# mathisbot/homomorph-rust

Hardware: AMD Instinct MI355X
Metric: homomorphic u32 ops/sec (add, mul) at d=dp=tau=128; 1/2/4/8 MI355X (higher is better)
Workload: dtype u32

## Files before the change

homomorph-rust_amd/csrc/adder_mfma.hip:

```cpp
#include <hip/hip_runtime.h>

#include "mfma_gf2.h"

namespace hm {

#ifdef HM_MFMA_PROFILE
constexpr int kMfmaProfSlots = 8;
__device__ unsigned long long *g_mfma_prof;
#define HM_PT(v) const unsigned long long v = __builtin_amdgcn_s_memtime()
#define HM_PACC(k, a, b) prof[k] += (b) - (a)
#else
#define HM_PT(v)
#define HM_PACC(k, a, b)
#endif

#ifndef HM_MFMA_PREFETCH
#define HM_MFMA_PREFETCH 3
#endif
#ifndef HM_MFMA_PREFETCH25
#define HM_MFMA_PREFETCH25 4
#endif
template <int NC> constexpr int kPrefetchOf = NC > 16 ? HM_MFMA_PREFETCH25 : NC <= 8 ? 2 : HM_MFMA_PREFETCH;
template <int NC> constexpr int kStage(int k) { return NC <= 8 ? 2 * k : 1 + 3 * k; }
template <int NC, class Side, int kPrefetch = kPrefetchOf<NC>>
__device__ __forceinline__ v16f tile_mfma(const v8i (&Af)[NC], uint32_t rb, uint32_t rbn,
                                          u32x4 (&pf)[kPrefetch], v16f acc, Side &&side) {
    static_assert(NC - kPrefetch > kStage<NC>(2), "next tile's B reads must follow its ring fill (stage 2)");
    u32x4 bq[NC];
#pragma unroll
    for (int c = 0; c < kPrefetch; ++c) bq[c] = pf[c];
#pragma unroll
    for (int c = 0; c < NC; ++c) {
        if (c + kPrefetch < NC) bq[c + kPrefetch] = lds_at<const u32x4>(rb)[2 * (c + kPrefetch)];
        else pf[c + kPrefetch - NC] = lds_at<const u32x4>(rbn)[2 * (c + kPrefetch - NC)];
        const v8i Bf = {(int)bq[c].x, (int)bq[c].y, (int)bq[c].z, (int)bq[c].w, 0, 0, 0, 0};
        acc = mfma_fp4(Af[c], Bf, acc);
        asm volatile("" : "+v"(acc)::"memory");
        if (c == kStage<NC>(0)) side(0);
        if (c == kStage<NC>(1)) side(1);
        if (c == kStage<NC>(2)) side(2);
    }
    return acc;
}

constexpr uint32_t kPhaseBytes = 16u * 32u;

#ifndef HM_REC_WAIT_YOUNG
#define HM_REC_WAIT_YOUNG 0
#endif
__device__ __forceinline__ void wait_record(int young) {
    if (!HM_REC_WAIT_YOUNG || young <= 0) asm volatile("s_waitcnt vmcnt(0)" ::: "memory");
    else if (young >= 16) asm volatile("s_waitcnt vmcnt(16)" ::: "memory");
    else if (young >= 8) asm volatile("s_waitcnt vmcnt(8)" ::: "memory");
    else if (young >= 4) asm volatile("s_waitcnt vmcnt(4)" ::: "memory");
    else if (young >= 2) asm volatile("s_waitcnt vmcnt(2)" ::: "memory");
    else asm volatile("s_waitcnt vmcnt(1)" ::: "memory");
}

__device__ __forceinline__ void sum_store(uint64_t base, uint32_t off, uint32_t v) {
    asm volatile("global_store_dword %0, %1, %2" : : "v"(off), "v"(v), "s"(base) : "memory");
}

constexpr int kGetregHwId = 4 | 31 << 11;
constexpr int kGetregWaveSlot = 4 | 3 << 11;
constexpr int kGetregXccId = 20 | 3 << 11;

#ifndef HM_CHAIN_PRIO
#define HM_CHAIN_PRIO 2
#endif
static_assert(HM_CHAIN_PRIO == 0 || HM_CHAIN_PRIO == 2, "HM_CHAIN_PRIO: 0 (by age) or 2 (rotating levels)");
template <int NC> constexpr int kChainPrio = NC == 13 ? HM_CHAIN_PRIO : 0;
__device__ __forceinline__ void set_prio(uint32_t level) {
    if (level == 0) __builtin_amdgcn_s_setprio(0);
    else if (level == 1) __builtin_amdgcn_s_setprio(1);
    else if (level == 2) __builtin_amdgcn_s_setprio(2);
    else __builtin_amdgcn_s_setprio(3);
}

#ifndef HM_MFMA_WPB
#define HM_MFMA_WPB kAddWavesPerBlock
#endif
constexpr int kMfmaWpb = HM_MFMA_WPB;
static_assert(kMfmaWpb <= kAddWavesPerBlock, "host LDS plan");

template <int NC>
__global__ void __launch_bounds__(64 * kMfmaWpb)
__attribute__((amdgpu_waves_per_eu(MfmaCfg<NC>::kWavesPerEU, MfmaCfg<NC>::kWavesPerEU)))
add_chain_mfma_kernel(AddArgs A) {
#ifdef HM_MFMA_PROFILE
    const unsigned long long prof_rt0 = __builtin_amdgcn_s_memrealtime();
    const unsigned long long prof_st0 = __builtin_amdgcn_s_memtime();
#endif
    kt_start(A.kt);
    using Cfg = MfmaCfg<NC>;
    constexpr int kRevWords = Cfg::kRevWords, kRsWords = Cfg::kRsWords, kRec = Cfg::kRecWords;
    extern __shared__ uint32_t lds[];
    __shared__ uint32_t stage[kMfmaWpb][2][kRec];
    uint32_t *tab = lds;
    for (uint32_t k = threadIdx.x; k < 256; k += blockDim.x) {
        uint32_t v = 0u;
#pragma unroll
        for (int t = 0; t < 8; ++t) v |= ((k >> t) & 1u) << (4 * t + 1);
        tab[k] = v;
    }
    __syncthreads();
    const int wave = (int)rfl(threadIdx.x >> 6);
    const uint64_t e = (uint64_t)blockIdx.x * (blockDim.x >> 6) + wave;
    if (e >= A.n) {
        kt_finish(A.kt);
        return;
    }
    const int lane = lane_id();
    const uint32_t L = A.nbits;
    uint32_t *Ls = lds + 256 + (size_t)wave * A.chain_lds;
    uint32_t *C = Ls + Cfg::kHalo;
    uint32_t *ring = C + A.mf_cw;
    uint32_t *RS = ring + Cfg::kRingWords;
    const uint32_t *ws = A.ws + e * A.ws_stride;
    uint64_t *po = A.out.limbs + e * A.out.stride;
    uint32_t *dout = A.out.degree + e * L;
    const uint32_t oP = A.cntX, oAB = oP + A.cntP, oD = oAB + A.cntAB;
    auto rec_word = [&](uint32_t u, uint32_t &base, uint32_t &step) {
        const uint32_t offD = L * (A.cntAB + A.cntP);
        if (u < oP) base = offD + 2 * L + u, step = A.cntX;
        else if (u < oAB) base = L * A.cntAB + (u - oP), step = A.cntP;
        else if (u < oD) base = u - oAB, step = A.cntAB;
        else if (u == oD + 1) base = offD, step = 1;
        else base = offD + L, step = 1;
    };
    uint32_t lbase, lstep, lbase2 = 0, lstep2 = 0;
    rec_word((uint32_t)lane, lbase, lstep);
    if constexpr (kRec > 64) rec_word(64u + (uint32_t)lane, lbase2, lstep2);
    const bool two = kRec > 64 && oD + 2 > 64;
    const uint64_t wsu = ((uint64_t)rfl((uint32_t)((uintptr_t)ws >> 32)) << 32) |
                         rfl((uint32_t)(uintptr_t)ws);
    auto stage_rec = [&](uint32_t i) {
        const uint32_t voff = 4u * (lbase + i * lstep);
        const uint32_t m0 = (uint32_t)(uintptr_t)&stage[wave][i & 1][0];
        asm volatile("s_mov_b32 m0, %2\n\ts_nop 0\n\tglobal_load_lds_dword %0, %1"
                     :
                     : "v"(voff), "s"(wsu), "s"(m0)
                     : "memory", "m0");
        if (two) {
            const uint32_t voff2 = 4u * (lbase2 + i * lstep2);
            asm volatile("s_mov_b32 m0, %2\n\ts_nop 0\n\tglobal_load_lds_dword %0, %1"
                         :
                         : "v"(voff2), "s"(wsu), "s"(m0 + 256u)
                         : "memory", "m0");
        }
    };
    stage_rec(0);
    constexpr int kPrio = kChainPrio<NC>;
    uint32_t slot = 0u;
    if constexpr (kPrio == 2) slot = __builtin_amdgcn_s_getreg(kGetregWaveSlot);

#ifdef HM_MFMA_PROFILE
    unsigned long long prof[4] = {0, 0, 0, 0};
#endif
    for (uint32_t k = lane; k < Cfg::kHalo + A.mf_cw; k += kWave) Ls[k] = 0u;
    for (int k = 4 * kRevWords + lane; k < kRsWords; k += kWave) RS[k] = 0u;
    wsync();
    int nc = 0;
    int degc = -1;
    int tw = -1;
    int young = 0;
    uint32_t offo = 0;
    for (uint32_t i = 0; i < L; ++i) {
        HM_PT(tw0);
        if constexpr (kPrio == 2) set_prio((slot + i) & 3u);
        wait_record(young);
        young = 0;
        const uint32_t *rec = &stage[wave][i & 1][0];
        HM_PT(t0);
        HM_PACC(3, tw0, t0);
        if (tw < 0) {
            store_sum_x(rec, (int)A.cntX, C, nc, po + offo, A.ob.b[i], dout + i, A.status);
        } else {
            const int capw = 2 * (int)cap_of(A.ob.b[i]);
            uint32_t *so = (uint32_t *)(po + offo);
            int ldeg = -1;
            if (lane < 32) {
                const uint32_t v = (lane < (int)A.cntX ? rec[lane] : 0u) ^ C[lane];
                if (lane < capw) so[lane] = v;
                if (v) ldeg = lane * 32 + 31 - (int)__builtin_clz(v);
            }
            for (int w = tw + lane; w < capw; w += kWave) so[w] = 0u;
            int deg = wave_max_i32(ldeg);
            if (nc > 32) deg = degc;
            if (lane == 0) {
                if (deg > (int)A.ob.b[i]) flag(A.status, HM_ERR_CAPACITY);
                dout[i] = (uint32_t)max(deg, 0);
            }
        }
        offo += cap_of(A.ob.b[i]);
        HM_PT(t1);
        HM_PACC(0, t0, t1);
        if (i + 1 == L) break;
        const int np = bitwords((int)rfl(rec[oD])), nab = bitwords((int)rfl(rec[oD + 1]));
        const uint32_t *abi = rec + oAB;
        wsync();
        if (np == 0 || nc == 0) {
            const int n = max(nc, nab);
            for (int w = lane; w < n; w += kWave) C[w] = w < nab ? abi[w] : 0u;
            nc = nab;
            degc = (int)rfl(rec[oD + 1]) - 1;
            tw = -1;
            wsync();
            stage_rec(i + 1);
            continue;
        }
        const uint32_t *pi = rec + oP;
        for (int k = lane; k < 4 * kRevWords; k += kWave) {
            const int q = kRevWords - 1 - (k >> 2);
            const uint32_t rev = __builtin_bitreverse32(q < np ? pi[q] : 0u);
            RS[k] = tab[(rev >> (8 * (k & 3))) & 0xFFu];
        }
        wsync();
        stage_rec(i + 1);
        const int D = np;
        const int lane = lane_opaque(), col = lane & 31, h = lane >> 5;
        v8i Af[NC];
        const int jb = 32 * (kRevWords - D + h) - 1 - row_bit(col);
        const uint32_t rw0 = lds_opaque(lds_addr(RS) + 4u * (uint32_t)(jb >> 3));
        const uint32_t sh = 4u * (uint32_t)(jb & 7);
#pragma unroll
        for (int c = 0; c < NC; ++c) {
            const HM_LDS uint32_t *rw = lds_at<const uint32_t>(rw0) + 8 * c;
            const uint32_t w0 = rw[0], w1 = rw[1], w2 = rw[2], w3 = rw[3], w4 = rw[4];
            Af[c] = (v8i){(int)funnel(w1, w0, sh), (int)funnel(w2, w1, sh), (int)funnel(w3, w2, sh),
                          (int)funnel(w4, w3, sh), 0, 0, 0, 0};
        }
        HM_PT(t2);
        HM_PACC(1, t1, t2);
        const int nout = max(nc + np, nab);
        const int tiles = (nout + 31) >> 5;
        const uint64_t sonv = (uint64_t)(uintptr_t)(po + offo);
        const uint64_t son = ((uint64_t)rfl((uint32_t)(sonv >> 32)) << 32) | rfl((uint32_t)sonv);
        const int capn = 2 * (int)cap_of(A.ob.b[i + 1]);
        const int wlo = 32;
        int ldeg = -1;
        const int alg = (int)rfl(rec[oD]) - 1 + degc;
        const bool track = alg <= (int)rfl(rec[oD + 1]) - 1;
        v16f acc;
#pragma unroll
        for (int j = 0; j < 16; ++j) acc[j] = 8388608.0f;
        uint32_t gprev = 0u;
        const uint32_t rb0 = lds_opaque(lds_addr(ring) + 16u * (uint32_t)(col + h));
        const uint32_t put0 = lds_opaque(lds_addr(ring) + 8u * (uint32_t)lane);
        uint32_t cF = lds_opaque(lds_addr(C) + 4u * (uint32_t)(32 * (tiles - 2) - D + (lane >> 1)) +
                                 2u * (uint32_t)(lane & 1));
        uint32_t cW = lds_opaque(lds_addr(C) + 4u * (uint32_t)(32 * (tiles - 1) + col));
        const uint32_t col4 = 4u * (uint32_t)col;
        auto rbase = [&](int T) { return rb0 + kPhaseBytes * (uint32_t)(T & 3); };
        {
            constexpr int kPasses = (32 + 2 * NC + 31) / 32;
            uint32_t f0[kPasses], f1[kPasses];
#pragma unroll
            for (int p = 0; p < kPasses; ++p) {
                f0[p] = lds_at<const uint8_t>(cF)[128 * (p + 1)];
                f1[p] = lds_at<const uint8_t>(cF)[128 * (p + 1) + 1];
            }
#pragma unroll
            for (int p = 0; p < kPasses; ++p) f0[p] = tab[f0[p]], f1[p] = tab[f1[p]];
#pragma unroll
            for (int p = 0; p < kPasses; ++p) {
                const uint32_t ph = kPhaseBytes * (uint32_t)((tiles - 1 + p) & 3);
                const u32x2 fn = {f0[p], f1[p]};
                *lds_at<u32x2>(put0 + ph) = fn;
                if (ph < 16u * (uint32_t)Cfg::kMirror) *lds_at<u32x2>(put0 + ph + 16u * kMfmaRingSlots) = fn;
            }
        }
        wsync();
        constexpr int kPrefetch = kPrefetchOf<NC>;
        u32x4 pf[kPrefetch];
#pragma unroll
        for (int c = 0; c < kPrefetch; ++c) pf[c] = lds_at<const u32x4>(rbase(tiles - 1))[2 * c];
        uint32_t rb = rbase(tiles - 1);
        uint32_t abw = 0u;
        for (int T = tiles - 1; T >= 0; --T) {
            wsync();
            if constexpr (NC > 16) rb = rbase(T);
            const uint32_t ph = kPhaseBytes * (uint32_t)((T - 1) & 3);
            const uint32_t rbn = rb0 + ph;
            const uint32_t pp = put0 + ph;
            const bool mirror = ph < 16u * (uint32_t)Cfg::kMirror;
            uint32_t f0, f1;
            u32x2 fn;
            if (32 * T < nab) {
                asm volatile("" ::: "memory");
                const int W = 32 * T + (lane_opaque() & 31);
                abw = W < nab ? abi[W] : 0u;
            }
            if constexpr (kPrio == 0) __builtin_amdgcn_s_setprio(1);
            acc = tile_mfma<NC>(Af, rb, rbn, pf, acc, [&](int stage) {
                if (stage == 0) {
                    f0 = lds_at<const uint8_t>(cF)[0], f1 = lds_at<const uint8_t>(cF)[1];
                } else if (stage == 1) {
                    asm volatile("" : "+v"(f0), "+v"(f1));
                    fn.x = tab[f0], fn.y = tab[f1];
                } else {
                    asm volatile("" : "+v"(fn));
                    *lds_at<u32x2>(pp) = fn;
                    if (mirror) *lds_at<u32x2>(pp + 16u * kMfmaRingSlots) = fn;
                }
            });
            if constexpr (kPrio == 0) __builtin_amdgcn_s_setprio(0);
            const uint32_t tnow = acc_parities_hi16(acc);
            const uint32_t t = (tnow ^ gprev) >> (16 - 16 * h);
            const auto sw = __builtin_amdgcn_permlane32_swap(t, gprev, false, false);
            gprev = tnow;
            const uint32_t word = sw[0] | sw[1];
            const uint32_t v = word ^ abw;
            const bool full = T >= 1 && 32 * T + 32 <= capn;
            young += full ? 1 : 0;
            if (h == 0) {
                *lds_at<uint32_t>(cW) = v;
                const uint64_t sT = son + 128u * (uint32_t)T;
                if (full) {
                    sum_store(sT, col4, v);
                } else {
                    const int W = 32 * T + (lane_opaque() & 31);
                    if (W >= wlo && W < capn) sum_store(sT, col4, v);
                }
            }
            if (track) {
                asm volatile("" ::: "memory");
                const int Wq = 32 * T + (lane_opaque() & 31);
                if (h == 0 && v) ldeg = max(ldeg, Wq * 32 + 31 - (int)__builtin_clz(v));
            }
            rb = rbn;
            cF -= 128u;
            cW -= 128u;
        }
        const int deg = track ? wave_max_i32(ldeg) : alg;
        nc = deg >= 0 ? (deg >> 5) + 1 : 0;
        degc = deg;
        tw = 32 * tiles;
        wsync();
        HM_PT(t3);
        HM_PACC(2, t2, t3);
    }
#ifdef HM_MFMA_PROFILE
    if (lane == 0) {
        unsigned long long *g = g_mfma_prof + e * kMfmaProfSlots;
        for (int k = 0; k < 4; ++k) g[k] = prof[k];
        g[4] = prof_rt0, g[5] = __builtin_amdgcn_s_memrealtime();
        g[6] = __builtin_amdgcn_s_memtime() - prof_st0;
        g[7] = (unsigned long long)__builtin_amdgcn_s_getreg(kGetregXccId) << 32 | __builtin_amdgcn_s_getreg(kGetregHwId);
    }
#endif
    kt_finish(A.kt);
}

int launch_add_chain_mfma(const AddArgs &a, void *stream) {
    const int wpb = kMfmaWpb;
    const uint64_t blocks = (a.n + wpb - 1) / wpb;
    const size_t lds = (256 + (size_t)a.chain_lds * wpb) * 4;
#define HM_LAUNCH_CHAIN(NCV)                                                                      \
    hipLaunchKernelGGL((add_chain_mfma_kernel<NCV>), dim3((unsigned)blocks), dim3(64 * wpb), lds,  \
                       (hipStream_t)stream, a)
    if (a.mfma == MfmaCfg<7>::kChunks) HM_LAUNCH_CHAIN(7);
    else if (a.mfma == MfmaCfg<13>::kChunks) HM_LAUNCH_CHAIN(13);
    else if (a.mfma == MfmaCfg<25>::kChunks) HM_LAUNCH_CHAIN(25);
    else return -1;
#undef HM_LAUNCH_CHAIN
    return hipGetLastError() == hipSuccess ? 0 : -1;
}

}
```

Measured before the change: 9.703 million.

## Batch chain-head LDS loads and RS build ahead of tile loop for non-13 widths

Moves the per-iteration tile loop into a lambda and adds a new head path, used for every NC except 13 unless HM_CHAIN_HEAD13 is set. The new head issues the record, C, P-word and carry-ring loads up front in batches and builds RS from registers with a fixed pass count. It also loads the A-fragment words before the funnel shifts so LDS latency overlaps with other work. The write-back of the previous sum now goes through sum_store, and NC==13 keeps the old sequential path. The new path adds register pressure and extra wave syncs.

Result: no change. 9.702 million (-0.0%).

```diff
diff --git a/homomorph-rust_amd/csrc/adder_mfma.hip b/homomorph-rust_amd/csrc/adder_mfma.hip
--- a/homomorph-rust_amd/csrc/adder_mfma.hip
+++ b/homomorph-rust_amd/csrc/adder_mfma.hip
@@ -76,6 +76,11 @@
     else if (level == 2) __builtin_amdgcn_s_setprio(2);
     else __builtin_amdgcn_s_setprio(3);
 }
+
+#ifndef HM_CHAIN_HEAD13
+#define HM_CHAIN_HEAD13 0
+#endif
+template <int NC> constexpr bool kBatchedHead = NC == 13 ? HM_CHAIN_HEAD13 != 0 : true;
 
 #ifndef HM_MFMA_WPB
 #define HM_MFMA_WPB kAddWavesPerBlock
@@ -168,91 +173,109 @@
     for (uint32_t i = 0; i < L; ++i) {
         HM_PT(tw0);
         if constexpr (kPrio == 2) set_prio((slot + i) & 3u);
-        wait_record(young);
-        young = 0;
-        const uint32_t *rec = &stage[wave][i & 1][0];
-        HM_PT(t0);
-        HM_PACC(3, tw0, t0);
-        if (tw < 0) {
-            store_sum_x(rec, (int)A.cntX, C, nc, po + offo, A.ob.b[i], dout + i, A.status);
-        } else {
-            const int capw = 2 * (int)cap_of(A.ob.b[i]);
-            uint32_t *so = (uint32_t *)(po + offo);
+        constexpr int kPrefetch = kPrefetchOf<NC>;
+        auto run_tiles = [&](const v8i (&Af)[NC], u32x4 (&pf)[kPrefetch], const uint32_t *abi, int nab, int tiles,
+                             uint64_t son, int capn, int alg, bool track, uint32_t rb0, uint32_t put0,
+                             uint32_t cF, uint32_t cW, uint32_t col4, int h) {
+            HM_PT(t2);
+            const int wlo = 32;
             int ldeg = -1;
-            if (lane < 32) {
-                const uint32_t v = (lane < (int)A.cntX ? rec[lane] : 0u) ^ C[lane];
-                if (lane < capw) so[lane] = v;
-                if (v) ldeg = lane * 32 + 31 - (int)__builtin_clz(v);
-            }
-            for (int w = tw + lane; w < capw; w += kWave) so[w] = 0u;
-            int deg = wave_max_i32(ldeg);
-            if (nc > 32) deg = degc;
-            if (lane == 0) {
-                if (deg > (int)A.ob.b[i]) flag(A.status, HM_ERR_CAPACITY);
-                dout[i] = (uint32_t)max(deg, 0);
-            }
-        }
-        offo += cap_of(A.ob.b[i]);
-        HM_PT(t1);
-        HM_PACC(0, t0, t1);
-        if (i + 1 == L) break;
-        const int np = bitwords((int)rfl(rec[oD])), nab = bitwords((int)rfl(rec[oD + 1]));
-        const uint32_t *abi = rec + oAB;
-        wsync();
-        if (np == 0 || nc == 0) {
-            const int n = max(nc, nab);
-            for (int w = lane; w < n; w += kWave) C[w] = w < nab ? abi[w] : 0u;
-            nc = nab;
-            degc = (int)rfl(rec[oD + 1]) - 1;
-            tw = -1;
-            wsync();
-            stage_rec(i + 1);
-            continue;
-        }
-        const uint32_t *pi = rec + oP;
-        for (int k = lane; k < 4 * kRevWords; k += kWave) {
-            const int q = kRevWords - 1 - (k >> 2);
-            const uint32_t rev = __builtin_bitreverse32(q < np ? pi[q] : 0u);
-            RS[k] = tab[(rev >> (8 * (k & 3))) & 0xFFu];
-        }
-        wsync();
-        stage_rec(i + 1);
-        const int D = np;
-        const int lane = lane_opaque(), col = lane & 31, h = lane >> 5;
-        v8i Af[NC];
-        const int jb = 32 * (kRevWords - D + h) - 1 - row_bit(col);
-        const uint32_t rw0 = lds_opaque(lds_addr(RS) + 4u * (uint32_t)(jb >> 3));
-        const uint32_t sh = 4u * (uint32_t)(jb & 7);
-#pragma unroll
-        for (int c = 0; c < NC; ++c) {
-            const HM_LDS uint32_t *rw = lds_at<const uint32_t>(rw0) + 8 * c;
-            const uint32_t w0 = rw[0], w1 = rw[1], w2 = rw[2], w3 = rw[3], w4 = rw[4];
-            Af[c] = (v8i){(int)funnel(w1, w0, sh), (int)funnel(w2, w1, sh), (int)funnel(w3, w2, sh),
-                          (int)funnel(w4, w3, sh), 0, 0, 0, 0};
-        }
-        HM_PT(t2);
-        HM_PACC(1, t1, t2);
-        const int nout = max(nc + np, nab);
-        const int tiles = (nout + 31) >> 5;
-        const uint64_t sonv = (uint64_t)(uintptr_t)(po + offo);
-        const uint64_t son = ((uint64_t)rfl((uint32_t)(sonv >> 32)) << 32) | rfl((uint32_t)sonv);
-        const int capn = 2 * (int)cap_of(A.ob.b[i + 1]);
-        const int wlo = 32;
-        int ldeg = -1;
-        const int alg = (int)rfl(rec[oD]) - 1 + degc;
-        const bool track = alg <= (int)rfl(rec[oD + 1]) - 1;
-        v16f acc;
-#pragma unroll
-        for (int j = 0; j < 16; ++j) acc[j] = 8388608.0f;
-        uint32_t gprev = 0u;
-        const uint32_t rb0 = lds_opaque(lds_addr(ring) + 16u * (uint32_t)(col + h));
-        const uint32_t put0 = lds_opaque(lds_addr(ring) + 8u * (uint32_t)lane);
-        uint32_t cF = lds_opaque(lds_addr(C) + 4u * (uint32_t)(32 * (tiles - 2) - D + (lane >> 1)) +
-                                 2u * (uint32_t)(lane & 1));
-        uint32_t cW = lds_opaque(lds_addr(C) + 4u * (uint32_t)(32 * (tiles - 1) + col));
-        const uint32_t col4 = 4u * (uint32_t)col;
-        auto rbase = [&](int T) { return rb0 + kPhaseBytes * (uint32_t)(T & 3); };
-        {
+            v16f acc;
+#pragma unroll
+            for (int j = 0; j < 16; ++j) acc[j] = 8388608.0f;
+            uint32_t gprev = 0u;
+            auto rbase = [&](int T) { return rb0 + kPhaseBytes * (uint32_t)(T & 3); };
+            uint32_t rb = rbase(tiles - 1);
+            uint32_t abw = 0u;
+            for (int T = tiles - 1; T >= 0; --T) {
+                wsync();
+                if constexpr (NC > 16) rb = rbase(T);
+                const uint32_t ph = kPhaseBytes * (uint32_t)((T - 1) & 3);
+                const uint32_t rbn = rb0 + ph;
+                const uint32_t pp = put0 + ph;
+                const bool mirror = ph < 16u * (uint32_t)Cfg::kMirror;
+                uint32_t f0, f1;
+                u32x2 fn;
+                if (32 * T < nab) {
+                    asm volatile("" ::: "memory");
+                    const int W = 32 * T + (lane_opaque() & 31);
+                    abw = W < nab ? abi[W] : 0u;
+                }
+                if constexpr (kPrio == 0) __builtin_amdgcn_s_setprio(1);
+                acc = tile_mfma<NC>(Af, rb, rbn, pf, acc, [&](int stage) {
+                    if (stage == 0) {
+                        f0 = lds_at<const uint8_t>(cF)[0], f1 = lds_at<const uint8_t>(cF)[1];
+                    } else if (stage == 1) {
+                        asm volatile("" : "+v"(f0), "+v"(f1));
+                        fn.x = tab[f0], fn.y = tab[f1];
+                    } else {
+                        asm volatile("" : "+v"(fn));
+                        *lds_at<u32x2>(pp) = fn;
+                        if (mirror) *lds_at<u32x2>(pp + 16u * kMfmaRingSlots) = fn;
+                    }
+                });
+                if constexpr (kPrio == 0) __builtin_amdgcn_s_setprio(0);
+                const uint32_t tnow = acc_parities_hi16(acc);
+                const uint32_t t = (tnow ^ gprev) >> (16 - 16 * h);
+                const auto sw = __builtin_amdgcn_permlane32_swap(t, gprev, false, false);
+                gprev = tnow;
+                const uint32_t word = sw[0] | sw[1];
+                const uint32_t v = word ^ abw;
+                const bool full = T >= 1 && 32 * T + 32 <= capn;
+                young += full ? 1 : 0;
+                if (h == 0) {
+                    *lds_at<uint32_t>(cW) = v;
+                    const uint64_t sT = son + 128u * (uint32_t)T;
+                    if (full) {
+                        sum_store(sT, col4, v);
+                    } else {
+                        const int W = 32 * T + (lane_opaque() & 31);
+                        if (W >= wlo && W < capn) sum_store(sT, col4, v);
+                    }
+                }
+                if (track) {
+                    asm volatile("" ::: "memory");
+                    const int Wq = 32 * T + (lane_opaque() & 31);
+                    if (h == 0 && v) ldeg = max(ldeg, Wq * 32 + 31 - (int)__builtin_clz(v));
+                }
+                rb = rbn;
+                cF -= 128u;
+                cW -= 128u;
+            }
+            const int deg = track ? wave_max_i32(ldeg) : alg;
+            nc = deg >= 0 ? (deg >> 5) + 1 : 0;
+            degc = deg;
+            tw = 32 * tiles;
+            wsync();
+            HM_PT(t3);
+            HM_PACC(2, t2, t3);
+        };
+        if constexpr (kBatchedHead<NC>) {
+            uint32_t obi = A.ob.b[i], obn = A.ob.b[i + 1 < L ? i + 1 : i];
+            wait_record(young);
+            asm volatile("" : "+s"(obi), "+s"(obn));
+            young = 0;
+            const uint32_t *rec = &stage[wave][i & 1][0];
+            const uint32_t *pi = rec + oP, *abi = rec + oAB;
+            HM_PT(t0);
+            HM_PACC(3, tw0, t0);
+            if (tw < 0) store_sum_x(rec, (int)A.cntX, C, nc, po + offo, obi, dout + i, A.status);
+            const int lane = lane_opaque(), col = lane & 31, h = lane >> 5;
+            const uint32_t dPv = rec[oD], dABv = rec[oD + 1];
+            const uint32_t xr = rec[col], cr = C[col];
+            constexpr int kRsPasses = (4 * kRevWords + kWave - 1) / kWave;
+            static_assert(kWave * kRsPasses <= kRsWords, "RS passes stay inside RS");
+            const int q0 = kRevWords - 1 - (lane >> 2);
+            uint32_t pw[kRsPasses];
+#pragma unroll
+            for (int t = 0; t < kRsPasses; ++t) pw[t] = pi[max(q0 - 16 * t, 0)];
+            const int dP = (int)rfl(dPv), dAB = (int)rfl(dABv);
+            const int np = bitwords(dP), nab = bitwords(dAB);
+            const int D = np;
+            const int nout = max(nc + np, nab);
+            const int tiles = (nout + 31) >> 5;
+            uint32_t cF = lds_opaque(lds_addr(C) + 4u * (uint32_t)(32 * (tiles - 2) - D + (lane >> 1)) +
+                                     2u * (uint32_t)(lane & 1));
             constexpr int kPasses = (32 + 2 * NC + 31) / 32;
             uint32_t f0[kPasses], f1[kPasses];
 #pragma unroll
@@ -260,8 +283,49 @@
                 f0[p] = lds_at<const uint8_t>(cF)[128 * (p + 1)];
                 f1[p] = lds_at<const uint8_t>(cF)[128 * (p + 1) + 1];
             }
+            if (tw >= 0) {
+                const int capw = 2 * (int)cap_of(obi);
+                const uint64_t sov = (uint64_t)(uintptr_t)(po + offo);
+                const uint64_t so = ((uint64_t)rfl((uint32_t)(sov >> 32)) << 32) | rfl((uint32_t)sov);
+                const uint32_t v = (col < (int)A.cntX ? xr : 0u) ^ cr;
+                if (lane < 32 && lane < capw) sum_store(so, 4u * (uint32_t)lane, v);
+                for (int w = tw; w < capw; w += kWave)
+                    if (w + lane < capw) sum_store(so + 4u * (uint32_t)w, 4u * (uint32_t)lane, 0u);
+                int deg = degc;
+                if (nc <= (int)A.cntX) deg = wave_max_i32(lane < 32 && v ? lane * 32 + 31 - (int)__builtin_clz(v) : -1);
+                if (deg > (int)obi && lane == 0) flag(A.status, HM_ERR_CAPACITY);
+                if (lane == 0) dout[i] = (uint32_t)max(deg, 0);
+            }
+            offo += cap_of(obi);
+            HM_PT(t1);
+            HM_PACC(0, t0, t1);
+            if (i + 1 == L) break;
+            wsync();
+            if (np == 0 || nc == 0) {
+                const int n = max(nc, nab);
+                for (int w = lane; w < n; w += kWave) C[w] = w < nab ? abi[w] : 0u;
+                nc = nab;
+                degc = dAB - 1;
+                tw = -1;
+                wsync();
+                stage_rec(i + 1);
+                continue;
+            }
+            uint32_t rs[kRsPasses];
+#pragma unroll
+            for (int t = 0; t < kRsPasses; ++t) {
+                const uint32_t rev = __builtin_bitreverse32((uint32_t)(q0 - 16 * t) < (uint32_t)np ? pw[t] : 0u);
+                rs[t] = tab[(rev >> (8 * (lane & 3))) & 0xFFu];
+            }
 #pragma unroll
             for (int p = 0; p < kPasses; ++p) f0[p] = tab[f0[p]], f1[p] = tab[f1[p]];
+            const uint32_t rsw = lds_opaque(lds_addr(RS) + 4u * (uint32_t)lane);
+#pragma unroll
+            for (int t = 0; t < kRsPasses; ++t) lds_at<uint32_t>(rsw)[kWave * t] = rs[t];
+            wsync();
+            stage_rec(i + 1);
+            const uint32_t rb0 = lds_opaque(lds_addr(ring) + 16u * (uint32_t)(col + h));
+            const uint32_t put0 = lds_opaque(lds_addr(ring) + 8u * (uint32_t)lane);
 #pragma unroll
             for (int p = 0; p < kPasses; ++p) {
                 const uint32_t ph = kPhaseBytes * (uint32_t)((tiles - 1 + p) & 3);
@@ -269,76 +333,135 @@
                 *lds_at<u32x2>(put0 + ph) = fn;
                 if (ph < 16u * (uint32_t)Cfg::kMirror) *lds_at<u32x2>(put0 + ph + 16u * kMfmaRingSlots) = fn;
             }
+            wsync();
+            v8i Af[NC];
+            const int jb = 32 * (kRevWords - D + h) - 1 - row_bit(col);
+            const uint32_t rw0 = lds_opaque(lds_addr(RS) + 4u * (uint32_t)(jb >> 3));
+            const uint32_t sh = 4u * (uint32_t)(jb & 7);
+            uint32_t aw[NC][5];
+#pragma unroll
+            for (int c = 0; c < NC; ++c)
+#pragma unroll
+                for (int t = 0; t < 5; ++t) aw[c][t] = lds_at<const uint32_t>(rw0)[8 * c + t];
+            u32x4 pf[kPrefetch];
+#pragma unroll
+            for (int c = 0; c < kPrefetch; ++c) pf[c] = lds_at<const u32x4>(rb0 + kPhaseBytes * (uint32_t)((tiles - 1) & 3))[2 * c];
+#pragma unroll
+            for (int c = 0; c < NC; ++c)
+                Af[c] = (v8i){(int)funnel(aw[c][1], aw[c][0], sh), (int)funnel(aw[c][2], aw[c][1], sh),
+                              (int)funnel(aw[c][3], aw[c][2], sh), (int)funnel(aw[c][4], aw[c][3], sh), 0, 0, 0, 0};
+            const uint64_t sonv = (uint64_t)(uintptr_t)(po + offo);
+            const uint64_t son = ((uint64_t)rfl((uint32_t)(sonv >> 32)) << 32) | rfl((uint32_t)sonv);
+            const int capn = 2 * (int)cap_of(obn);
+            const int alg = dP - 1 + degc;
+            const bool track = alg <= dAB - 1;
+            uint32_t cW = lds_opaque(lds_addr(C) + 4u * (uint32_t)(32 * (tiles - 1) + col));
+            const uint32_t col4 = 4u * (uint32_t)col;
+            HM_PT(t2);
+            HM_PACC(1, t1, t2);
+            run_tiles(Af, pf, abi, nab, tiles, son, capn, alg, track, rb0, put0, cF, cW, col4, h);
+        } else {
+            wait_record(young);
+            young = 0;
+            const uint32_t *rec = &stage[wave][i & 1][0];
+            HM_PT(t0);
+            HM_PACC(3, tw0, t0);
+            if (tw < 0) {
+                store_sum_x(rec, (int)A.cntX, C, nc, po + offo, A.ob.b[i], dout + i, A.status);
+            } else {
+                const int capw = 2 * (int)cap_of(A.ob.b[i]);
+                uint32_t *so = (uint32_t *)(po + offo);
+                int ldeg = -1;
+                if (lane < 32) {
+                    const uint32_t v = (lane < (int)A.cntX ? rec[lane] : 0u) ^ C[lane];
+                    if (lane < capw) so[lane] = v;
+                    if (v) ldeg = lane * 32 + 31 - (int)__builtin_clz(v);
+                }
+                for (int w = tw + lane; w < capw; w += kWave) so[w] = 0u;
+                int deg = wave_max_i32(ldeg);
+                if (nc > 32) deg = degc;
+                if (lane == 0) {
+                    if (deg > (int)A.ob.b[i]) flag(A.status, HM_ERR_CAPACITY);
+                    dout[i] = (uint32_t)max(deg, 0);
+                }
+            }
+            offo += cap_of(A.ob.b[i]);
+            HM_PT(t1);
+            HM_PACC(0, t0, t1);
+            if (i + 1 == L) break;
+            const int np = bitwords((int)rfl(rec[oD])), nab = bitwords((int)rfl(rec[oD + 1]));
+            const uint32_t *abi = rec + oAB;
+            wsync();
+            if (np == 0 || nc == 0) {
+                const int n = max(nc, nab);
+                for (int w = lane; w < n; w += kWave) C[w] = w < nab ? abi[w] : 0u;
+                nc = nab;
+                degc = (int)rfl(rec[oD + 1]) - 1;
+                tw = -1;
+                wsync();
+                stage_rec(i + 1);
+                continue;
+            }
+            const uint32_t *pi = rec + oP;
+            for (int k = lane; k < 4 * kRevWords; k += kWave) {
+                const int q = kRevWords - 1 - (k >> 2);
+                const uint32_t rev = __builtin_bitreverse32(q < np ? pi[q] : 0u);
+                RS[k] = tab[(rev >> (8 * (k & 3))) & 0xFFu];
+            }
+            wsync();
+            stage_rec(i + 1);
+            const int D = np;
+            const int lane = lane_opaque(), col = lane & 31, h = lane >> 5;
+            v8i Af[NC];
+            const int jb = 32 * (kRevWords - D + h) - 1 - row_bit(col);
+            const uint32_t rw0 = lds_opaque(lds_addr(RS) + 4u * (uint32_t)(jb >> 3));
+            const uint32_t sh = 4u * (uint32_t)(jb & 7);
+#pragma unroll
+            for (int c = 0; c < NC; ++c) {
+                const HM_LDS uint32_t *rw = lds_at<const uint32_t>(rw0) + 8 * c;
+                const uint32_t w0 = rw[0], w1 = rw[1], w2 = rw[2], w3 = rw[3], w4 = rw[4];
+                Af[c] = (v8i){(int)funnel(w1, w0, sh), (int)funnel(w2, w1, sh), (int)funnel(w3, w2, sh),
+                              (int)funnel(w4, w3, sh), 0, 0, 0, 0};
+            }
+            const int nout = max(nc + np, nab);
+            const int tiles = (nout + 31) >> 5;
+            const uint64_t sonv = (uint64_t)(uintptr_t)(po + offo);
+            const uint64_t son = ((uint64_t)rfl((uint32_t)(sonv >> 32)) << 32) | rfl((uint32_t)sonv);
+            const int capn = 2 * (int)cap_of(A.ob.b[i + 1]);
+            const int alg = (int)rfl(rec[oD]) - 1 + degc;
+            const bool track = alg <= (int)rfl(rec[oD + 1]) - 1;
+            const uint32_t rb0 = lds_opaque(lds_addr(ring) + 16u * (uint32_t)(col + h));
+            const uint32_t put0 = lds_opaque(lds_addr(ring) + 8u * (uint32_t)lane);
+            uint32_t cF = lds_opaque(lds_addr(C) + 4u * (uint32_t)(32 * (tiles - 2) - D + (lane >> 1)) +
+                                     2u * (uint32_t)(lane & 1));
+            uint32_t cW = lds_opaque(lds_addr(C) + 4u * (uint32_t)(32 * (tiles - 1) + col));
+            const uint32_t col4 = 4u * (uint32_t)col;
+            {
+                constexpr int kPasses = (32 + 2 * NC + 31) / 32;
+                uint32_t f0[kPasses], f1[kPasses];
+#pragma unroll
+                for (int p = 0; p < kPasses; ++p) {
+                    f0[p] = lds_at<const uint8_t>(cF)[128 * (p + 1)];
+                    f1[p] = lds_at<const uint8_t>(cF)[128 * (p + 1) + 1];
+                }
+#pragma unroll
+                for (int p = 0; p < kPasses; ++p) f0[p] = tab[f0[p]], f1[p] = tab[f1[p]];
+#pragma unroll
+                for (int p = 0; p < kPasses; ++p) {
+                    const uint32_t ph = kPhaseBytes * (uint32_t)((tiles - 1 + p) & 3);
+                    const u32x2 fn = {f0[p], f1[p]};
+                    *lds_at<u32x2>(put0 + ph) = fn;
+                    if (ph < 16u * (uint32_t)Cfg::kMirror) *lds_at<u32x2>(put0 + ph + 16u * kMfmaRingSlots) = fn;
+                }
+            }
+            wsync();
+            u32x4 pf[kPrefetch];
+#pragma unroll
+            for (int c = 0; c < kPrefetch; ++c) pf[c] = lds_at<const u32x4>(rb0 + kPhaseBytes * (uint32_t)((tiles - 1) & 3))[2 * c];
+            HM_PT(t2);
+            HM_PACC(1, t1, t2);
+            run_tiles(Af, pf, abi, nab, tiles, son, capn, alg, track, rb0, put0, cF, cW, col4, h);
         }
-        wsync();
-        constexpr int kPrefetch = kPrefetchOf<NC>;
-        u32x4 pf[kPrefetch];
-#pragma unroll
-        for (int c = 0; c < kPrefetch; ++c) pf[c] = lds_at<const u32x4>(rbase(tiles - 1))[2 * c];
-        uint32_t rb = rbase(tiles - 1);
-        uint32_t abw = 0u;
-        for (int T = tiles - 1; T >= 0; --T) {
-            wsync();
-            if constexpr (NC > 16) rb = rbase(T);
-            const uint32_t ph = kPhaseBytes * (uint32_t)((T - 1) & 3);
-            const uint32_t rbn = rb0 + ph;
-            const uint32_t pp = put0 + ph;
-            const bool mirror = ph < 16u * (uint32_t)Cfg::kMirror;
-            uint32_t f0, f1;
-            u32x2 fn;
-            if (32 * T < nab) {
-                asm volatile("" ::: "memory");
-                const int W = 32 * T + (lane_opaque() & 31);
-                abw = W < nab ? abi[W] : 0u;
-            }
-            if constexpr (kPrio == 0) __builtin_amdgcn_s_setprio(1);
-            acc = tile_mfma<NC>(Af, rb, rbn, pf, acc, [&](int stage) {
-                if (stage == 0) {
-                    f0 = lds_at<const uint8_t>(cF)[0], f1 = lds_at<const uint8_t>(cF)[1];
-                } else if (stage == 1) {
-                    asm volatile("" : "+v"(f0), "+v"(f1));
-                    fn.x = tab[f0], fn.y = tab[f1];
-                } else {
-                    asm volatile("" : "+v"(fn));
-                    *lds_at<u32x2>(pp) = fn;
-                    if (mirror) *lds_at<u32x2>(pp + 16u * kMfmaRingSlots) = fn;
-                }
-            });
-            if constexpr (kPrio == 0) __builtin_amdgcn_s_setprio(0);
-            const uint32_t tnow = acc_parities_hi16(acc);
-            const uint32_t t = (tnow ^ gprev) >> (16 - 16 * h);
-            const auto sw = __builtin_amdgcn_permlane32_swap(t, gprev, false, false);
-            gprev = tnow;
-            const uint32_t word = sw[0] | sw[1];
-            const uint32_t v = word ^ abw;
-            const bool full = T >= 1 && 32 * T + 32 <= capn;
-            young += full ? 1 : 0;
-            if (h == 0) {
-                *lds_at<uint32_t>(cW) = v;
-                const uint64_t sT = son + 128u * (uint32_t)T;
-                if (full) {
-                    sum_store(sT, col4, v);
-                } else {
-                    const int W = 32 * T + (lane_opaque() & 31);
-                    if (W >= wlo && W < capn) sum_store(sT, col4, v);
-                }
-            }
-            if (track) {
-                asm volatile("" ::: "memory");
-                const int Wq = 32 * T + (lane_opaque() & 31);
-                if (h == 0 && v) ldeg = max(ldeg, Wq * 32 + 31 - (int)__builtin_clz(v));
-            }
-            rb = rbn;
-            cF -= 128u;
-            cW -= 128u;
-        }
-        const int deg = track ? wave_max_i32(ldeg) : alg;
-        nc = deg >= 0 ? (deg >> 5) + 1 : 0;
-        degc = deg;
-        tw = 32 * tiles;
-        wsync();
-        HM_PT(t3);
-        HM_PACC(2, t2, t3);
     }
 #ifdef HM_MFMA_PROFILE
     if (lane == 0) {
```
